# simdjson/simdjson-java

Hardware: AMD Instinct MI355X
Metric: GB/s JSON scanned (stage-1) (higher is better)
Workload: dtype u8; 1 GPU; twitter.json x6801 concatenated (north-star '4 GiB concatenated twitter.json'): stage-1 = UTF-8 validation + structural indexing + uint32 index compaction, one fused single-pass kernel; index count and status checked before and after the timed steps (the whole array against the oracle's closed form: --full); bytes_per_gpu=4294933515, structurals_per_gpu=375843663, tile_steps=auto, preheat_launches=40

## Files before the change

simdjson-java_amd/csrc/stage1.hip:

```cpp
#include <hip/hip_runtime.h>
#include <hip/hip_ext.h>
#include <stdint.h>

#include <type_traits>

#include "sj_block.h"
#include "sj_block32.h"
#include "sj_chain.h"
#include "stage1.h"

namespace sjmi {

__host__ __device__ constexpr uint32_t msad_const(int k, int base_weight_log2) {
    uint32_t r = 0;
    for (int i = 0; i < 4; ++i) {
        const int wgt = 1 << (base_weight_log2 + i);
        const int v = (1 << k) + wgt <= 255 ? (1 << k) + wgt : (1 << k) - wgt;
        r |= (uint32_t)v << (8 * i);
    }
    return r;
}

template <int K>
__device__ __forceinline__ sj_u64 plane_msad(const uint32_t w[16]) {
    constexpr uint32_t bit = 0x01010101u << K;
    constexpr uint32_t cA = msad_const(K, 0), cB = msad_const(K, 4);
    uint32_t half[2];
#pragma unroll
    for (int h = 0; h < 2; ++h) {
        uint32_t acc = 0;
#pragma unroll
        for (int j = 0; j < 4; ++j) {
            uint32_t v = __builtin_amdgcn_msad_u8(cA, w[8 * h + 2 * j] & bit, 0u);
            v = __builtin_amdgcn_msad_u8(cB, w[8 * h + 2 * j + 1] & bit, v);
            acc |= v << (8 * j);
        }
        half[h] = acc;
    }
    return (sj_u64)half[0] | ((sj_u64)half[1] << 32);
}

__device__ __forceinline__ void transpose_fast(const uint32_t w[16], sj_u64 p[8]) {
    p[0] = plane_msad<0>(w);
    p[1] = plane_msad<1>(w);
    p[2] = plane_msad<2>(w);
    p[3] = plane_msad<3>(w);
    p[4] = plane_msad<4>(w);
    p[5] = plane_msad<5>(w);
    p[6] = plane_msad<6>(w);
    p[7] = plane_msad<7>(w);
}

__global__ void k_transpose_selftest(const uint32_t* __restrict__ words, uint32_t nblocks, uint32_t* mismatches) {
    const uint32_t b = blockIdx.x * blockDim.x + threadIdx.x;
    if (b >= nblocks) return;
    uint32_t w[16];
#pragma unroll
    for (int i = 0; i < 16; ++i) w[i] = words[b * 16 + i];
    sj_u64 pf[8], pb[8], pr[8];
    transpose_fast(w, pf);
    sj_transpose_butterfly(w, pb);
    sj_transpose_ref(w, pr);
    uint32_t bad = 0;
#pragma unroll
    for (int k = 0; k < 8; ++k) bad += (pf[k] != pr[k]) + (pb[k] != pr[k]);
    if (bad) atomicAdd(mismatches, bad);
}

__device__ __forceinline__ uint32_t wave_sum(uint32_t v) {
#pragma unroll
    for (int d = 32; d >= 1; d >>= 1) v += __shfl_xor(v, d);
    return v;
}

__device__ __forceinline__ void publish_aggregate(sj_u64* tile_state, uint32_t tile, uint32_t T0, uint32_t T1,
                                                  uint32_t tpar, uint32_t errbits = 0) {
    granule_store(&tile_state[tile], CHAIN_AGG | ((sj_u64)errbits << 41) | ((sj_u64)tpar << 40) | ((sj_u64)T1 << 20) | (sj_u64)T0);
}
__device__ __forceinline__ void publish_prefix(sj_u64* tile_state, uint32_t tile, uint32_t par_after, sj_u64 cnt_after) {
    granule_store(&tile_state[tile], CHAIN_PFX | ((sj_u64)par_after << 40) | cnt_after);
}


template <int K>
__device__ __forceinline__ void tile_lookback(const sj_u64* tile_state, uint32_t tile, int lane, uint32_t* par_in,
                                              sj_u64* cnt_in, Stage1Result* res) {
    sj_u64 g0 = 0, g1 = 0;
    uint32_t gpar = 0;
    long long k = (long long)tile;
    uint32_t P = 0;
    sj_u64 C = 0;
    for (;;) {
        const long long hi = k - 1 - (long long)lane * K;
        sj_u64 v[K];
        int jp = K;
        int J = 64;
        for (uint32_t spins = 0;; ++spins) {
#pragma unroll
            for (int j = 0; j < K; ++j) v[j] = (hi - j >= 0) ? granule_load(&tile_state[hi - j]) : CHAIN_PFX;
            jp = K;
#pragma unroll
            for (int j = K - 1; j >= 0; --j)
                if ((v[j] >> 62) == 2) jp = j;
            bool ready = true;
#pragma unroll
            for (int j = 0; j < K; ++j)
                if (j < jp && v[j] == 0) ready = false;
            const sj_u64 pm = __ballot(jp < K);
            J = pm ? __builtin_ctzll(pm) : 64;
            const sj_u64 need = J >= 63 ? ~0ull : ((2ull << J) - 1ull);
            if ((__ballot(ready) & need) == need) break;
            if (spins > CHAIN_SPIN_LIMIT) {
                if (lane == 0)
                    __hip_atomic_fetch_or(&res->status, SJMI_ST_INTERNAL, __ATOMIC_RELAXED, __HIP_MEMORY_SCOPE_AGENT);
                break;
            }
            __builtin_amdgcn_s_sleep(1);
        }
        const int nin = lane < J ? K : (lane == J ? jp : 0);
        uint32_t c0 = 0, c1 = 0, lpar = 0;
        sj_u64 pfxv = 0;
#pragma unroll
        for (int j = K - 1; j >= 0; --j) {
            if (j == jp) pfxv = v[j];
            if (j < nin) {
                const uint32_t a0 = (uint32_t)v[j] & 0xFFFFFu, a1 = (uint32_t)(v[j] >> 20) & 0xFFFFFu;
                const uint32_t n0 = c0 + (lpar ? a1 : a0), n1 = c1 + (lpar ? a0 : a1);
                c0 = n0;
                c1 = n1;
                lpar ^= (uint32_t)(v[j] >> 40) & 1u;
            }
        }
        const sj_u64 pb = __ballot(lpar);
        const uint32_t q = (lane < 63) ? (uint32_t)__popcll(pb >> (lane + 1)) & 1u : 0u;
        const uint32_t w0 = wave_sum(q ? c1 : c0);
        const uint32_t w1 = wave_sum(q ? c0 : c1);
        const uint32_t wpar = (uint32_t)__popcll(pb) & 1u;
        if (J < 64) {
            const sj_u64 pv = __shfl(pfxv, J);
            P = (uint32_t)(pv >> 40) & 1u;
            C = pv & ((1ull << 40) - 1ull);
            C += P ? w1 : w0;
            P ^= wpar;
            C += P ? g1 : g0;
            P ^= gpar;
            break;
        }
        const sj_u64 n0 = (sj_u64)w0 + (wpar ? g1 : g0);
        const sj_u64 n1 = (sj_u64)w1 + (wpar ? g0 : g1);
        g0 = n0;
        g1 = n1;
        gpar ^= wpar;
        k -= 64 * K;
    }
    *par_in = P;
    *cnt_in = C;
}

__device__ __forceinline__ void single_doc_setup(const Stage1Single& ss, sj_u64 len, sj_u64 count, uint32_t status) {
    if (!ss.index_offsets) return;
    ss.doc_offsets[0] = 0;
    ss.doc_offsets[1] = len;
    ss.index_offsets[0] = 0;
    ss.index_offsets[1] = (status & (SJMI_ST_CAPACITY | SJMI_ST_INTERNAL)) ? 0ull : count;
    ss.doc_status[0] = status & 0xFFu;
    ss.doc_str_offsets[0] = 0;
    ss.doc_str_offsets[1] = 0;
    for (int i = 0; i < (int)(sizeof(WalkResult) / 4); ++i) ss.walk_result[i] = 0;
    for (int i = 0; i < 16; ++i) ss.slow_header[i] = 0;
}

constexpr int SCAN_K = 4;
struct Stage1Chain {
    static constexpr int K = SCAN_K;
    uint32_t* err;
    Stage1Result* res;
    uint32_t* out;
    sj_u64 out_cap;
    Stage1Result* result_out;
    const Stage1Single& ss;
    sj_u64 len;

    __device__ static void fold(const sj_u64 (&v)[K], uint32_t* c0, uint32_t* c1, uint32_t* par) {
        uint32_t a = 0, b = 0, lp = 0;
#pragma unroll
        for (int j = 0; j < K; ++j) {
            const uint32_t a0 = (uint32_t)v[j] & 0xFFFFFu, a1 = (uint32_t)(v[j] >> 20) & 0xFFFFFu;
            const uint32_t n0 = a + (lp ? a1 : a0), n1 = b + (lp ? a0 : a1);
            a = n0;
            b = n1;
            lp ^= (uint32_t)(v[j] >> 40) & 1u;
        }
        *c0 = a;
        *c1 = b;
        *par = lp;
    }
    __device__ static uint32_t errors(const sj_u64 (&v)[K], uint32_t q) {
        uint32_t e = 0;
#pragma unroll
        for (int j = 0; j < K; ++j) {
            if ((v[j] >> 41) & 1u) e |= SJMI_ST_UTF8;
            if ((v[j] >> 44) & 1u) e |= SJMI_ST_HALO;
            if ((v[j] >> (42 + q)) & 1u) e |= SJMI_ST_UNESCAPED;
            q ^= (uint32_t)(v[j] >> 40) & 1u;
        }
        return e;
    }
    __device__ void report(uint32_t e) const {
        if (__ballot(e != 0)) {
#pragma unroll
            for (int d = 32; d >= 1; d >>= 1) e |= __shfl_xor(e, d);
            if ((threadIdx.x & 63) == 0) __hip_atomic_fetch_or(err, e, __ATOMIC_RELAXED, __HIP_MEMORY_SCOPE_WORKGROUP);
        }
    }
    __device__ static void publish(const sj_u64 (&v)[K], sj_u64* pfx, sj_u64 first, uint32_t n, uint32_t q, sj_u64 run) {
#pragma unroll
        for (int j = 0; j < K; ++j) {
            run += q ? (uint32_t)(v[j] >> 20) & 0xFFFFFu : (uint32_t)v[j] & 0xFFFFFu;
            q ^= (uint32_t)(v[j] >> 40) & 1u;
            if (first + j < n) publish_prefix(pfx, (uint32_t)(first + j), q, run);
        }
    }

    struct Window {
        sj_u64 pb;
        uint32_t qrel;
        uint32_t mine0, mine1;
        uint32_t incl0, incl1;
        uint32_t tot0, tot1;
    };
    __device__ Window window(const sj_u64 (&v)[K], int lane) const {
        Window w;
        uint32_t c0, c1, lp;
        fold(v, &c0, &c1, &lp);
        w.pb = __ballot(lp);
        w.qrel = (uint32_t)__popcll(w.pb & ((1ull << lane) - 1ull)) & 1u;
        w.mine0 = w.qrel ? c1 : c0;
        w.mine1 = w.qrel ? c0 : c1;
        w.incl0 = wave_incl_add(w.mine0);
        w.incl1 = wave_incl_add(w.mine1);
        w.tot0 = (uint32_t)__builtin_amdgcn_readlane((int)w.incl0, 63);
        w.tot1 = (uint32_t)__builtin_amdgcn_readlane((int)w.incl1, 63);
        return w;
    }
    __device__ ChainState advance(ChainState in, const sj_u64 (&v)[K], const Window& w) const {
        report(errors(v, in.w ^ w.qrel));
        return {in.w ^ ((uint32_t)__popcll(w.pb) & 1u), in.c + (in.w ? w.tot1 : w.tot0)};
    }
    __device__ void publish_window(const sj_u64 (&v)[K], sj_u64* pfx, sj_u64 first, uint32_t n, ChainState in, const Window& w) const {
        publish(v, pfx, first, n, in.w ^ w.qrel, in.c + (in.w ? w.incl1 - w.mine1 : w.incl0 - w.mine0));
    }
    __device__ ChainState publish_ready(const sj_u64 (&v)[K], sj_u64* pfx, sj_u64 first, uint32_t n, int lane, bool act,
                                        ChainState s) const {
        uint32_t c0, c1, lp;
        fold(v, &c0, &c1, &lp);
        const sj_u64 pb = __ballot(act && lp);
        const uint32_t q = s.w ^ ((uint32_t)__popcll(pb & ((1ull << lane) - 1ull)) & 1u);
        const uint32_t mine = act ? (q ? c1 : c0) : 0u;
        const uint32_t incl = wave_incl_add(mine);
        if (act) publish(v, pfx, first, n, q, s.c + (incl - mine));
        report(act ? errors(v, q) : 0u);
        return {s.w ^ ((uint32_t)__popcll(pb) & 1u), s.c + (uint32_t)__builtin_amdgcn_readlane((int)incl, 63)};
    }
    __device__ void give_up() const {
        __hip_atomic_fetch_or(&res->status, SJMI_ST_INTERNAL, __ATOMIC_RELAXED, __HIP_MEMORY_SCOPE_AGENT);
        if (result_out) {
            result_out->count = 0;
            result_out->status = SJMI_ST_INTERNAL;
            result_out->reserved = 0;
            single_doc_setup(ss, len, 0, SJMI_ST_INTERNAL);
        }
    }
    __device__ void finish(ChainState s) const {
        res->count = s.c;
        uint32_t e = __hip_atomic_load(err, __ATOMIC_RELAXED, __HIP_MEMORY_SCOPE_WORKGROUP);
        if (s.w) e |= SJMI_ST_UNCLOSED;
        if (s.c < out_cap) out[s.c] = 0;
        else e |= SJMI_ST_CAPACITY;
        if (e) __hip_atomic_fetch_or(&res->status, e, __ATOMIC_RELAXED, __HIP_MEMORY_SCOPE_AGENT);
        if (result_out) {
            const uint32_t st_all = e | __hip_atomic_load(&res->status, __ATOMIC_RELAXED, __HIP_MEMORY_SCOPE_AGENT);
            result_out->count = s.c;
            result_out->status = st_all;
            result_out->reserved = 0;
            single_doc_setup(ss, len, s.c, st_all);
        }
    }
};


struct StepData {
    uint4 q0, q1, q2, q3;
    sj_u64 halo;
};

__device__ __forceinline__ void load_step(StepData& d, const uint8_t* __restrict__ buf, sj_u64 blk, sj_u64 nblocks, bool left_halo = false) {
    const sj_u64 b = blk < nblocks ? blk : nblocks - 1;
    const uint4* src = reinterpret_cast<const uint4*>(buf + b * 64);
    d.q0 = src[0];
    d.q1 = src[1];
    d.q2 = src[2];
    d.q3 = src[3];
    d.halo = *reinterpret_cast<const sj_u64*>(buf + ((b > 0 || left_halo) ? (long long)(b * 64) - 8 : 0ll));
}

constexpr uint32_t NO_TILE = 0xFFFFFFFFu;

__device__ __forceinline__ void zero_next_workspace(uint4* zero_ptr, uint32_t zero_chunks, uint32_t slot, uint32_t nslots,
                                                    int lane) {
    if (zero_ptr && nslots) {
        const uint32_t per = (zero_chunks + nslots - 1) / nslots;
        const uint32_t b = slot * per, e = b + per < zero_chunks ? b + per : zero_chunks;
        for (uint32_t i = b + (uint32_t)lane; i < e; i += 64) zero_ptr[i] = make_uint4(0, 0, 0, 0);
    }
}

constexpr uint32_t TICKET_CLASSES = 8;
constexpr int LB_K = 1;

#ifndef SJMI_S1_SORT_MIN
#define SJMI_S1_SORT_MIN 192
#endif
template <int S>
struct Parked {
    sj_u64 pot[S][64];
    sj_u64 m0[S][64];
    uint32_t meta[S][64];
};
template <int S, int LDSW>
union WaveShared {
    Parked<S> park;
    alignas(16) uint32_t stage[LDSW / 4];
    static_assert(sizeof(Parked<S>) <= LDSW, "LDS slice too small");
};

template <int S, int LDSW, bool SAFE, bool BATCH>
__device__ __forceinline__ void
stage1_body(const uint8_t* __restrict__ buf, sj_u64 len, uint32_t* __restrict__ out, sj_u64 out_cap,
            sj_u64* gstate, uint32_t* ticket, Stage1Result* res, uint32_t ngran, uint32_t dbg, uint4* zero_ptr,
            uint32_t zero_chunks, Stage1Result* result_out, sj_u64* __restrict__ blkpar, const uint32_t* __restrict__ skip,
            uint32_t* __restrict__ blkidx, uint16_t* __restrict__ blkw, uint4* zero2_ptr, uint32_t zero2_chunks, const Stage1Single& ss) {
    constexpr int E = S, CAP = LDSW / 4;
    if (skip && *skip) return;
    static_assert(S <= 4, "meta packs 14-bit offsets: at most 4 steps per granule");
    __shared__ WaveShared<S, LDSW> sh[4];
    __shared__ ChainHandoff hand;
    __shared__ uint32_t scan_err;
    const int lane = threadIdx.x & 63;
    const int wave = __builtin_amdgcn_readfirstlane(threadIdx.x >> 6);
    constexpr bool safe = SAFE;
    sj_u64* const agg = gstate;
    sj_u64* const pfx = gstate + ngran;
    const uint32_t my_cu = cu_id();
    uint32_t* const scanner_cu = reinterpret_cast<uint32_t*>(res) + WS_SCANNER_CU_WORD;
    if (!safe && blockIdx.x == 0) {
        if (threadIdx.x == 0) __hip_atomic_store(scanner_cu, my_cu, __ATOMIC_RELAXED, __HIP_MEMORY_SCOPE_AGENT);
        if ((dbg & DBG_FAKE_TIMEOUT) && threadIdx.x == 0)
            __hip_atomic_fetch_or(&res->status, SJMI_ST_INTERNAL, __ATOMIC_RELAXED, __HIP_MEMORY_SCOPE_AGENT);
        if (threadIdx.x == 0) {
            hand.seq = 0;
            hand.w = (dbg & FLAG_ENTRY_PARITY) ? 1u : 0u;
            hand.c = 0;
            scan_err = 0;
        }
        __syncthreads();
        if (!(dbg & DBG_NO_LOOKBACK)) {
            const Stage1Chain pol = {&scan_err, res, out, out_cap, result_out, ss, len};
            chain_scanner_wave(&hand, wave, lane, agg, pfx, ngran, pol);
        }
        return;
    }
    const uint32_t nworkers = (gridDim.x - (safe ? 0u : 1u)) * 4u;
    const uint32_t worker = (blockIdx.x - (safe ? 0u : 1u)) * 4u + (uint32_t)wave;
    WaveShared<S, LDSW>& ws = sh[wave];
    const uint32_t nblocks = (uint32_t)(len / 64) + ((dbg & FLAG_NO_TAIL) ? 0u : 1u);
    const uint32_t halo_blocks = dbg >> 16;
    const bool left_halo = halo_blocks != 0;
    const uint32_t entry_par = (dbg & FLAG_ENTRY_PARITY) ? 1u : 0u;
    const sj_u64 lt_mask = (1ull << lane) - 1ull;
    const uint32_t last = ngran - 1;

    const uint32_t NC = safe ? 1u : (nworkers < TICKET_CLASSES ? nworkers : TICKET_CLASSES);
    const uint32_t cls = worker % NC;
    uint32_t* const my_ticket = ticket + cls * 16u;
    uint32_t retire = 0;
    if (!safe && gridDim.x >= 64)
        retire = __hip_atomic_load(scanner_cu, __ATOMIC_RELAXED, __HIP_MEMORY_SCOPE_AGENT) ^ my_cu;
    else
        retire = 1;
    const bool first_by_ticket = safe || (dbg & FLAG_ALL_TICKETS) != 0;
    uint32_t cur;
    const uint32_t ticket_base = first_by_ticket ? 0u : (nworkers - cls + NC - 1u) / NC;
    if (first_by_ticket) cur = take_ticket(my_ticket) * NC + cls;
    else cur = worker;
    uint32_t prev = NO_TILE, prev_par = 0, prev_c0 = 0, prev_c1 = 0;
    uint32_t err = 0;
    StepData d;
    load_step(d, buf, cur * (64u * S) + (uint32_t)lane, nblocks, left_halo);

    for (;;) {
        const bool have = cur < ngran;
        uint32_t tk = 0;
        sj_u64 pfv = 0;
        sj_u64 pot[S], m[S];
        uint32_t meta[S];
        uint32_t wpar = 0, W0 = 0, WP = 0;
        auto request_ticket = [&] {
            if (lane == 0 && retire != 0) {
                uint32_t z = 0;
                asm volatile("" : "+v"(z));
                tk = __hip_atomic_fetch_add(my_ticket + z, 1u, __ATOMIC_RELAXED, __HIP_MEMORY_SCOPE_AGENT);
            }
        };
        auto request_prefix = [&] {
            uint32_t z = 0;
            asm volatile("" : "+v"(z));
            pfv = granule_load(&pfx[prev != NO_TILE && prev != 0 ? prev - 1 : 0u] + z);
        };
        auto next_granule = [&] {
            return retire != 0 ? ((uint32_t)__builtin_amdgcn_readfirstlane((int)tk) + ticket_base) * NC + cls : NO_TILE;
        };

        if (have) {
            __builtin_amdgcn_s_setprio(2);
            const uint32_t blk0 = cur * (64u * S);
            sj_u64 sm[S];
            uint32_t fl[S];
            uint32_t slow = 0;
            bool halo_short = false;
#pragma unroll
            for (int s = 0; s < S; ++s) {
                const uint32_t blk = blk0 + (uint32_t)s * 64u + (uint32_t)lane;
                const uint32_t w[16] = {d.q0.x, d.q0.y, d.q0.z, d.q0.w, d.q1.x, d.q1.y, d.q1.z, d.q1.w,
                                        d.q2.x, d.q2.y, d.q2.z, d.q2.w, d.q3.x, d.q3.y, d.q3.z, d.q3.w};
                const sj_u64 halo = d.halo;
                uint32_t plo[8], phi[8];
                sj_transpose32(w, plo, phi);
                asm volatile("" ::"v"(halo) : "memory");
                if (s + 1 < S) load_step(d, buf, blk0 + (uint32_t)(s + 1) * 64u + (uint32_t)lane, nblocks, left_halo);
                if (s == S - 1 && !safe) {
                    request_ticket();
                    request_prefix();
                }
                asm volatile("" ::: "memory");
                pot[s] = 0;
                sm[s] = 0;
                fl[s] = 0;
                bool unresolved = false;
                if (blk < nblocks) {
                    const bool has_halo = blk > 0 || left_halo;
                    uint32_t e_in = 0, p_in = 0;
                    if (has_halo) unresolved = !sj_carry_from_halo(halo, &e_in, &p_in);
                    if (blk0 + (uint32_t)s * 64u + 63u >= nblocks - 1u) {
                        const sj_u64 rem = len - (sj_u64)blk * 64;
                        sj_mask_tail32(plo, phi, rem < 64 ? (uint32_t)rem : 64u);
                    }
                    const uint32_t halo_hi = has_halo ? (uint32_t)(halo >> 32) & 0x80808080u : 0u;
                    const bool need_utf8 = __ballot((plo[7] | phi[7] | halo_hi) != 0) != 0;
                    SjUtf8Lazy uc = {0, 0};
                    if (need_utf8 && has_halo) uc = sj_utf8_carry_lazy(halo);
                    const SjBlockMasks32 bm = sj_block32(plo, phi, e_in, p_in, uc, need_utf8, BATCH, [](uint32_t x) { return __ballot(x != 0) != 0; });
                    pot[s] = ((sj_u64)bm.pot.hi << 32) | bm.pot.lo;
                    sm[s] = ((sj_u64)bm.sm0.hi << 32) | bm.sm0.lo;
                    fl[s] = bm.qpar | (min(bm.ue0, 1u) << 1) | (min(bm.ue1, 1u) << 2) | (min(bm.utf8, 1u) << 3);
                    if (BATCH) blkw[blk] = (uint16_t)bm.words;
                }
                slow |= unresolved ? (1u << s) : 0u;
            }
            if (__ballot(slow != 0)) {
                for (int s = 0; s < S; ++s) {
                    if (!((slow >> s) & 1u)) continue;
                    const sj_u64 blk = blk0 + (sj_u64)s * 64 + lane;
                    const sj_u64 start = blk * 64;
                    uint32_t w[16];
                    for (int i = 0; i < 16; ++i) w[i] = reinterpret_cast<const uint32_t*>(buf + start)[i];
                    const sj_u64 halo = *reinterpret_cast<const sj_u64*>(buf + start - 8);
                    uint32_t e_in = 0, p_in = 0;
                    sj_carry_slow(buf - (sj_u64)halo_blocks * 64, 0, start + (sj_u64)halo_blocks * 64, &e_in, &p_in);
                    if (left_halo && !(dbg & FLAG_HALO_FROM_START)) {
                        const uint8_t* hb = buf - (sj_u64)halo_blocks * 64;
                        const sj_u64 hs = start + (sj_u64)halo_blocks * 64;
                        if (sj_backslash_run_reaches(hb, 0, hb[hs - 1] == 0x22 ? hs - 1 : hs)) halo_short = true;
                    }
                    sj_u64 p[8];
                    sj_transpose_butterfly(w, p);
                    const sj_u64 rem = len - start;
                    sj_mask_tail(p, rem < 64 ? (uint32_t)rem : 64u);
                    const SjBlockMasks bm = sj_block(p, e_in, p_in, sj_utf8_carry(halo), true, nullptr, BATCH);
                    pot[s] = bm.pot;
                    sm[s] = bm.sm0;
                    fl[s] = bm.qpar | (bm.ue0 << 1) | (bm.ue1 << 2) | (bm.utf8 << 3);
                    if (BATCH && blk < nblocks) blkw[blk] = (uint16_t)bm.words;
                }
            }
            uint32_t gerr = 0;
#pragma unroll
            for (int s = 0; s < S; ++s) {
                const sj_u64 bal = __ballot(fl[s] & 1u);
                const uint32_t lp = ((uint32_t)__popcll(bal & lt_mask) & 1u) ^ wpar;
                wpar ^= (uint32_t)__popcll(bal) & 1u;
                m[s] = lp ? (pot[s] & sm[s]) : (pot[s] & ~sm[s]);
                const uint32_t c0 = (uint32_t)__popcll(m[s]), cp = (uint32_t)__popcll(pot[s]);
                const uint32_t packed = wave_incl_add(c0 | (cp << 16));
                const uint32_t tot = (uint32_t)__builtin_amdgcn_readlane((int)packed, 63);
                const uint32_t ex0 = W0 + (packed & 0xFFFFu) - c0;
                const uint32_t exp_ = WP + (packed >> 16) - cp;
                W0 += tot & 0xFFFFu;
                WP += tot >> 16;
                const uint32_t ue0 = (fl[s] >> 1) & 1u, ue1 = (fl[s] >> 2) & 1u;
                if (fl[s] & 8u) err |= SJMI_ST_UTF8;
                meta[s] = ex0 | (exp_ << 14) | ((lp ? ue1 : ue0) << 28) | ((lp ? ue0 : ue1) << 29) | (lp << 30);
                gerr |= ((fl[s] >> 3) & 1u) | ((meta[s] >> 27) & 6u);
            }
            uint32_t gbits = (__ballot(gerr & 1u) ? 1u : 0u) | (__ballot(gerr & 2u) ? 2u : 0u) | (__ballot(gerr & 4u) ? 4u : 0u);
            if (left_halo && __ballot(halo_short)) {
                gbits |= 8u;
                err |= SJMI_ST_HALO;
            }
            if (lane == 0 && !(dbg & DBG_NO_LOOKBACK)) {
                if (safe && cur == 0) publish_prefix(agg, 0, wpar ^ entry_par, (sj_u64)(entry_par ? WP - W0 : W0));
                else publish_aggregate(agg, cur, W0, WP - W0, wpar, gbits);
            }
            __builtin_amdgcn_s_setprio(0);
        }
        uint32_t nxt = NO_TILE;
        if (have) nxt = safe ? take_ticket(my_ticket) : next_granule();
        load_step(d, buf, nxt * (64u * S) + (uint32_t)lane, nblocks, left_halo);

        if (prev != NO_TILE) {
            uint32_t pe = entry_par;
            sj_u64 cnt_in = 0;
            if (dbg & DBG_NO_LOOKBACK) {
                cnt_in = (sj_u64)prev * 512ull * S;
            } else if (prev != 0) {
                if constexpr (safe) {
                    tile_lookback<LB_K>(agg, prev, lane, &pe, &cnt_in, res);
                } else {
                    sj_u64 pf = (sj_u64)(uint32_t)__builtin_amdgcn_readfirstlane((int)(uint32_t)pfv) |
                                ((sj_u64)(uint32_t)__builtin_amdgcn_readfirstlane((int)(uint32_t)(pfv >> 32)) << 32);
                    wait_prefix(&pfx[prev - 1], pf, [&] {
                        if (lane == 0) __hip_atomic_fetch_or(&res->status, SJMI_ST_INTERNAL, __ATOMIC_RELAXED, __HIP_MEMORY_SCOPE_AGENT);
                    });
                    pe = (uint32_t)(pf >> 40) & 1u;
                    cnt_in = pf & ((1ull << 40) - 1ull);
                }
            }
            const uint32_t WT_all = pe ? prev_c1 : prev_c0;
            if (safe && lane == 0 && !(dbg & DBG_NO_LOOKBACK)) {
                if (prev != 0) publish_prefix(agg, prev, pe ^ prev_par, cnt_in + WT_all);
                if (prev == last) {
                    const sj_u64 total = cnt_in + WT_all;
                    res->count = total;
                    uint32_t e = 0;
                    if (pe ^ prev_par) e |= SJMI_ST_UNCLOSED;
                    if (total < out_cap) out[total] = 0;
                    else e |= SJMI_ST_CAPACITY;
                    if (e) __hip_atomic_fetch_or(&res->status, e, __ATOMIC_RELAXED, __HIP_MEMORY_SCOPE_AGENT);
                }
            }
            const bool fits = cnt_in + WT_all < out_cap;
            if (!fits && WT_all) err |= SJMI_ST_CAPACITY;
            const sj_u64 pblk0 = (sj_u64)prev * (64 * S);
            uint32_t* stage = ws.stage;
#pragma unroll
            for (int g = 0; g < S / E; ++g) {
                sj_u64 mk[E];
                uint32_t pos[E];
                const uint32_t mb = ws.park.meta[g * E][0];
                const uint32_t gbase = pe ? ((mb >> 14) & 0x3FFFu) - (mb & 0x3FFFu) : (mb & 0x3FFFu);
                uint32_t gend = WT_all;
                if (g + 1 < S / E) {
                    const uint32_t me = ws.park.meta[(g + 1) * E][0];
                    gend = pe ? ((me >> 14) & 0x3FFFu) - (me & 0x3FFFu) : (me & 0x3FFFu);
                }
#pragma unroll
                for (int e = 0; e < E; ++e) {
                    const int s = g * E + e;
                    const sj_u64 pt = ws.park.pot[s][lane], mm = ws.park.m0[s][lane];
                    const uint32_t mt = ws.park.meta[s][lane];
                    mk[e] = pe ? (pt ^ mm) : mm;
                    const uint32_t o0 = mt & 0x3FFFu, op = (mt >> 14) & 0x3FFFu;
                    pos[e] = (pe ? op - o0 : o0) - gbase;
                    if (BATCH) blkidx[(pblk0 + (sj_u64)s * 64) + lane] = (uint32_t)(cnt_in + gbase) + pos[e];
                    if ((mt >> (28 + pe)) & 1u) err |= SJMI_ST_UNESCAPED;
                    if (blkpar) {
                        const sj_u64 pm = __ballot(((mt >> 30) ^ pe) & 1u);
                        if (lane == 0) blkpar[(sj_u64)prev * S + s] = pm;
                    }
                }
                wave_lds_fence();
                if (fits && !(dbg & DBG_NO_WRITE)) {
                    const uint32_t WT = gend - gbase;
                    uint32_t* dst0 = out + cnt_in + gbase;
                    auto flush_round = [&](uint32_t rbase, uint32_t rcount, uint32_t g0) {
                        const uint32_t span = g0 + rcount;
                        uint32_t* gbp = dst0 + rbase - g0;
                        for (uint32_t qi = lane; qi * 4 < span; qi += 64) {
                            const uint4 v = reinterpret_cast<const uint4*>(stage)[qi];
                            const uint32_t lo = qi * 4;
                            if (lo >= g0 && lo + 4 <= span) {
                                if constexpr (S == 4 && !BATCH) {
                                    typedef uint32_t u32x4_t __attribute__((ext_vector_type(4)));
                                    u32x4_t nv = {v.x, v.y, v.z, v.w};
                                    __builtin_nontemporal_store(nv, reinterpret_cast<u32x4_t*>(gbp) + qi);
                                } else {
                                    reinterpret_cast<uint4*>(gbp)[qi] = v;
                                }
                            } else {
                                if (lo + 0 >= g0 && lo + 0 < span) gbp[lo + 0] = v.x;
                                if (lo + 1 >= g0 && lo + 1 < span) gbp[lo + 1] = v.y;
                                if (lo + 2 >= g0 && lo + 2 < span) gbp[lo + 2] = v.z;
                                if (lo + 3 >= g0 && lo + 3 < span) gbp[lo + 3] = v.w;
                            }
                        }
                        wave_lds_fence();
                    };
                    auto fast_round = [&](uint32_t rbase, uint32_t rcount) {
                        const uint32_t g0 = (uint32_t)((cnt_in + gbase + rbase) & 3ull);
#pragma unroll
                        for (int e = 0; e < E; ++e) {
                            const uint32_t bstart = (uint32_t)((pblk0 + (sj_u64)(g * E + e) * 64 + lane) * 64);
                            uint32_t* q = stage + g0 + (pos[e] - rbase);
                            for (uint32_t lo = (uint32_t)mk[e]; lo; lo &= lo - 1) *q++ = bstart | (uint32_t)__builtin_ctz(lo);
                            for (uint32_t hi = (uint32_t)(mk[e] >> 32); hi; hi &= hi - 1)
                                *q++ = bstart | 32u | (uint32_t)__builtin_ctz(hi);
                        }
                        wave_lds_fence();
                        flush_round(rbase, rcount, g0);
                    };
                    auto sorted_round = [&](auto e0c, auto e1c, uint32_t rbase, uint32_t rcount) {
                        constexpr int E0 = decltype(e0c)::value, E1 = decltype(e1c)::value, NI = 2 * (E1 - E0);
                        static_assert(NI * 128 + 128 <= CAP, "the sort's tables overlay the staging slots");
                        const uint32_t g0 = (uint32_t)((cnt_in + gbase + rbase) & 3ull);
                        uint32_t* const hist = stage + NI * 128;
                        uint32_t* const bbase = hist + 64;
                        uint2* const items = reinterpret_cast<uint2*>(stage);
                        hist[lane] = 0u;
                        wave_lds_fence();
                        uint32_t hm[NI], cc[NI], rk[NI], inf[NI];
#pragma unroll
                        for (int e = E0; e < E1; ++e) {
                            const int i = 2 * (e - E0);
                            hm[i] = (uint32_t)mk[e];
                            hm[i + 1] = (uint32_t)(mk[e] >> 32);
                            cc[i] = (uint32_t)__popc(hm[i]);
                            cc[i + 1] = (uint32_t)__popc(hm[i + 1]);
                            const uint32_t p4 = (pos[e] - rbase + g0) * 4u;
                            const uint32_t ib = (uint32_t)(((g * E + e) * 64 + lane) * 64) << 16;
                            inf[i] = p4 | ib;
                            inf[i + 1] = (p4 + 4u * cc[i]) | (ib + (32u << 16));
                            rk[i] = atomicAdd(&hist[cc[i]], 1u);
                            rk[i + 1] = atomicAdd(&hist[cc[i + 1]], 1u);
                        }
                        wave_lds_fence();
                        const uint32_t hv = lane <= 32 ? hist[32 - lane] : 0u;
                        const uint32_t incl = wave_incl_add(hv);
                        if (lane <= 32) bbase[32 - lane] = incl - hv;
                        const uint32_t nz = (uint32_t)__builtin_amdgcn_readlane((int)incl, 31);
                        wave_lds_fence();
#pragma unroll
                        for (int i = 0; i < NI; ++i) items[bbase[cc[i]] + rk[i]] = make_uint2(hm[i], inf[i]);
                        wave_lds_fence();
                        const uint32_t trips = (nz + 63u) / 64u;
                        uint2 it[NI];
#pragma unroll
                        for (int r = 0; r < NI; ++r) it[r] = items[r * 64 + lane];
                        wave_lds_fence();
                        const uint32_t b32 = (uint32_t)(pblk0 * 64);
#pragma unroll
                        for (int r = 0; r < NI; ++r) {
                            if ((uint32_t)r >= trips) break;
                            uint32_t* q = reinterpret_cast<uint32_t*>(reinterpret_cast<char*>(stage) + (it[r].y & 0xFFFFu));
                            const uint32_t bv = b32 + (it[r].y >> 16);
                            uint32_t lo = it[r].x;
                            uint32_t* qh = q + __popc(lo) - 1;
                            while (lo) {
                                const uint32_t lz = (uint32_t)__builtin_clz(lo);
                                *q++ = bv | (uint32_t)__builtin_ctz(lo);
                                *qh-- = bv | (lz ^ 31u);
                                lo = lo & (lo - 1) & ~(0x80000000u >> lz);
                            }
                        }
                        wave_lds_fence();
                        flush_round(rbase, rcount, g0);
                    };
                    const uint32_t split = E >= 2 ? (uint32_t)__builtin_amdgcn_readfirstlane((int)pos[E / 2]) : 0u;
                    using std::integral_constant;
                    bool staged = false;
                    if (WT + 3 <= (uint32_t)CAP) {
                        if (WT > (uint32_t)(SJMI_S1_SORT_MIN * E)) sorted_round(integral_constant<int, 0>{}, integral_constant<int, E>{}, 0, WT);
                        else fast_round(0, WT);
                        staged = true;
                    }
                    if constexpr (E >= 2) {
                        if (!staged && split + 3 <= (uint32_t)CAP && WT - split + 3 <= (uint32_t)CAP) {
                            sorted_round(integral_constant<int, 0>{}, integral_constant<int, E / 2>{}, 0, split);
                            sorted_round(integral_constant<int, E / 2>{}, integral_constant<int, E>{}, split, WT - split);
                            staged = true;
                        }
                    }
                    if (!staged) {
                        for (uint32_t base = 0; base < WT; base += CAP) {
                            const uint32_t lim = base + CAP;
#pragma unroll
                            for (int e = 0; e < E; ++e) {
                                const uint32_t bstart = (uint32_t)((pblk0 + (sj_u64)(g * E + e) * 64 + lane) * 64);
                                uint32_t lo = (uint32_t)mk[e], hi = (uint32_t)(mk[e] >> 32);
                                uint32_t p2 = pos[e];
                                while (lo && p2 < lim) {
                                    stage[p2 - base] = bstart + (uint32_t)__builtin_ctz(lo);
                                    lo &= lo - 1;
                                    ++p2;
                                }
                                while (!lo && hi && p2 < lim) {
                                    stage[p2 - base] = bstart + 32u + (uint32_t)__builtin_ctz(hi);
                                    hi &= hi - 1;
                                    ++p2;
                                }
                                mk[e] = (sj_u64)lo | ((sj_u64)hi << 32);
                                pos[e] = p2;
                            }
                            wave_lds_fence();
                            const uint32_t nn = (WT - base) < (uint32_t)CAP ? (WT - base) : (uint32_t)CAP;
                            uint32_t* dst = dst0 + base;
                            for (uint32_t i = lane; i < nn; i += 64) dst[i] = stage[i];
                            wave_lds_fence();
                        }
                    }
                }
            }
        }
        if (!have) break;
        wave_lds_fence();
#pragma unroll
        for (int s = 0; s < S; ++s) {
            ws.park.pot[s][lane] = pot[s];
            ws.park.m0[s][lane] = m[s];
            ws.park.meta[s][lane] = meta[s];
        }
        wave_lds_fence();
        prev = cur;
        prev_par = wpar;
        prev_c0 = W0;
        prev_c1 = WP - W0;
        cur = nxt;
    }
#pragma unroll
    for (int dd = 32; dd >= 1; dd >>= 1) err |= __shfl_xor(err, dd);
    if (lane == 0 && err && !(dbg & DBG_NO_LOOKBACK))
        __hip_atomic_fetch_or(&res->status, err, __ATOMIC_RELAXED, __HIP_MEMORY_SCOPE_AGENT);
    zero_next_workspace(zero_ptr, zero_chunks, worker, nworkers, lane);
    zero_next_workspace(zero2_ptr, zero2_chunks, worker, nworkers, lane);
}

template <int S, int LDSW, bool SAFE, bool BATCH>
struct Stage1Kernel;
#ifndef SJMI_S1_PLAIN_WAVES
#define SJMI_S1_PLAIN_WAVES 4
#endif
template <int S, int LDSW, bool SAFE>
__global__ void __launch_bounds__(256)
#if SJMI_S1_PLAIN_WAVES
__attribute__((amdgpu_waves_per_eu(SJMI_S1_PLAIN_WAVES, SJMI_S1_PLAIN_WAVES)))
#endif
k_stage1(const uint8_t* __restrict__ buf, sj_u64 len, uint32_t* __restrict__ out, sj_u64 out_cap,
         sj_u64* gstate, uint32_t* ticket, Stage1Result* res, uint32_t ngran, uint32_t dbg, uint4* zero_ptr,
         uint32_t zero_chunks, Stage1Result* result_out, sj_u64* __restrict__ blkpar, const uint32_t* __restrict__ skip,
         uint32_t* __restrict__ blkidx, uint16_t* __restrict__ blkw, uint4* zero2_ptr, uint32_t zero2_chunks, Stage1Single ss) {
    stage1_body<S, LDSW, SAFE, false>(buf, len, out, out_cap, gstate, ticket, res, ngran, dbg, zero_ptr, zero_chunks, result_out, blkpar,
                                      skip, blkidx, blkw, zero2_ptr, zero2_chunks, ss);
}
#ifndef SJMI_S1_BATCH_WAVES
#define SJMI_S1_BATCH_WAVES 4
#endif
template <int S, int LDSW, bool SAFE>
__global__ void __launch_bounds__(256)
#if SJMI_S1_BATCH_WAVES
__attribute__((amdgpu_waves_per_eu(SJMI_S1_BATCH_WAVES, SJMI_S1_BATCH_WAVES)))
#endif
k_stage1_batch(const uint8_t* __restrict__ buf, sj_u64 len, uint32_t* __restrict__ out, sj_u64 out_cap,
               sj_u64* gstate, uint32_t* ticket, Stage1Result* res, uint32_t ngran, uint32_t dbg, uint4* zero_ptr,
               uint32_t zero_chunks, Stage1Result* result_out, sj_u64* __restrict__ blkpar, const uint32_t* __restrict__ skip,
               uint32_t* __restrict__ blkidx, uint16_t* __restrict__ blkw, uint4* zero2_ptr, uint32_t zero2_chunks, Stage1Single ss) {
    stage1_body<S, LDSW, SAFE, true>(buf, len, out, out_cap, gstate, ticket, res, ngran, dbg, zero_ptr, zero_chunks, result_out, blkpar,
                                     skip, blkidx, blkw, zero2_ptr, zero2_chunks, ss);
}
template <int S, int LDSW, bool SAFE>
struct Stage1Kernel<S, LDSW, SAFE, false> {
    static constexpr auto fn = k_stage1<S, LDSW, SAFE>;
};
template <int S, int LDSW, bool SAFE>
struct Stage1Kernel<S, LDSW, SAFE, true> {
    static constexpr auto fn = k_stage1_batch<S, LDSW, SAFE>;
};

static uint64_t granules_for(uint64_t len, int steps, bool no_tail = false) {
    const uint64_t nblocks = len / 64 + (no_tail ? 0 : 1);
    return (nblocks + 64ull * steps - 1) / (64ull * steps);
}

size_t stage1_workspace_bytes(uint64_t len, int steps) {
    return WS_TILE_STATE_OFFSET + 2 * (size_t)granules_for(len, steps) * sizeof(sj_u64);
}
Stage1Prefixes stage1_prefixes(const void* d_ws, uint64_t len, int steps) {
    Stage1Prefixes v;
    v.ngran = granules_for(len, steps);
    v.granule_bytes = (uint32_t)steps * 4096u;
    v.pfx = reinterpret_cast<const unsigned long long*>(static_cast<const uint8_t*>(d_ws) + WS_TILE_STATE_OFFSET) + v.ngran;
    return v;
}


int stage1_pick_steps(uint64_t len) {
    return len <= (4u << 20) ? 1 : (len <= (16u << 20) ? 2 : 4);
}

template <int S, int LDSW, bool SAFE, bool BATCH>
static hipError_t launch_mode(const uint8_t* d_buf, uint64_t len, uint32_t* d_out, uint64_t out_cap, sj_u64* gs,
                                 uint32_t* ticket, Stage1Result* res, uint64_t ngran, hipStream_t stream,
                                 hipEvent_t ev_start, hipEvent_t ev_stop, uint32_t dbg, const Stage1Extras& ex) {
    unsigned resident = 0;
    hipError_t e = resident_workgroups<Stage1Kernel<S, LDSW, SAFE, BATCH>::fn>(&resident);
    if (e != hipSuccess) return e;
    const uint64_t want = (ngran + 3) / 4 + (SAFE ? 0 : 1);
    if (dbg & DBG_SMALL_GRID) resident = SAFE ? 8 : 9;
    const dim3 grid((unsigned)(want < resident ? want : resident)), block(256);
    uint4* zp = static_cast<uint4*>(ex.zero_next);
    const uint32_t zc = (uint32_t)(ex.zero_bytes / 16);
    Stage1Result* ro = static_cast<Stage1Result*>(ex.result_out);
    sj_u64* bp = static_cast<sj_u64*>(ex.blkpar);
    uint32_t* bi = static_cast<uint32_t*>(ex.blkidx);
    uint16_t* bw = static_cast<uint16_t*>(ex.blkw);
    uint4* z2 = static_cast<uint4*>(ex.zero2);
    const uint32_t z2c = (uint32_t)(ex.zero2_bytes / 16);
    if (ev_start && ev_stop) {
        hipExtLaunchKernelGGL((Stage1Kernel<S, LDSW, SAFE, BATCH>::fn), grid, block, 0, stream, ev_start, ev_stop, 0, d_buf, (sj_u64)len,
                              d_out, (sj_u64)out_cap, gs, ticket, res, (uint32_t)ngran, dbg, zp, zc, ro, bp, ex.skip, bi, bw, z2, z2c, ex.single);
    } else {
        hipLaunchKernelGGL((Stage1Kernel<S, LDSW, SAFE, BATCH>::fn), grid, block, 0, stream, d_buf, (sj_u64)len, d_out, (sj_u64)out_cap,
                           gs, ticket, res, (uint32_t)ngran, dbg, zp, zc, ro, bp, ex.skip, bi, bw, z2, z2c, ex.single);
    }
    return hipGetLastError();
}

template <int S, int LDSW>
static hipError_t launch_variant(const uint8_t* d_buf, uint64_t len, uint32_t* d_out, uint64_t out_cap, sj_u64* gs,
                                 uint32_t* ticket, Stage1Result* res, uint64_t ngran, hipStream_t stream,
                                 hipEvent_t ev_start, hipEvent_t ev_stop, uint32_t dbg, const Stage1Extras& ex) {
    const bool batch = ex.blkidx && ex.blkw;
    if (dbg & FLAG_SAFE)
        return batch ? launch_mode<S, LDSW, true, true>(d_buf, len, d_out, out_cap, gs, ticket, res, ngran, stream, ev_start, ev_stop, dbg, ex)
                     : launch_mode<S, LDSW, true, false>(d_buf, len, d_out, out_cap, gs, ticket, res, ngran, stream, ev_start, ev_stop, dbg, ex);
    return batch ? launch_mode<S, LDSW, false, true>(d_buf, len, d_out, out_cap, gs, ticket, res, ngran, stream, ev_start, ev_stop, dbg, ex)
                 : launch_mode<S, LDSW, false, false>(d_buf, len, d_out, out_cap, gs, ticket, res, ngran, stream, ev_start, ev_stop, dbg, ex);
}

size_t stage1_block_entries(uint64_t len) { return (size_t)((len / 64 + 1 + 255) / 256 + 1) * 256; }

hipError_t stage1_launch(const uint8_t* d_buf, uint64_t len, uint32_t* d_out, uint64_t out_cap, void* d_ws,
                         int steps, hipStream_t stream, hipEvent_t ev_start, hipEvent_t ev_stop, uint32_t dbg, const Stage1Extras& ex) {
    const uint64_t ngran = granules_for(len, steps, (dbg & FLAG_NO_TAIL) != 0);
    if (ngran == 0) return hipErrorInvalidValue;
    const size_t ws_bytes = WS_TILE_STATE_OFFSET + 2 * (size_t)ngran * sizeof(sj_u64);
    hipError_t e = hipSuccess;
    if (!ex.workspace_is_zero && (e = hipMemsetAsync(d_ws, 0, ws_bytes, stream)) != hipSuccess) return e;
    uint8_t* ws = static_cast<uint8_t*>(d_ws);
    uint32_t* ticket = reinterpret_cast<uint32_t*>(ws + WS_TICKET_OFFSET);
    Stage1Result* res = reinterpret_cast<Stage1Result*>(ws + WS_RESULT_OFFSET);
    sj_u64* gs = reinterpret_cast<sj_u64*>(ws + WS_TILE_STATE_OFFSET);
    switch (steps) {
    case 1: e = launch_variant<1, 6144>(d_buf, len, d_out, out_cap, gs, ticket, res, ngran, stream, ev_start, ev_stop, dbg, ex); break;
    case 2: e = launch_variant<2, 9216>(d_buf, len, d_out, out_cap, gs, ticket, res, ngran, stream, ev_start, ev_stop, dbg, ex); break;
    case 4: e = launch_variant<4, 9216>(d_buf, len, d_out, out_cap, gs, ticket, res, ngran, stream, ev_start, ev_stop, dbg, ex); break;
    default: return hipErrorInvalidValue;
    }
    return e;
}

hipError_t transpose_selftest_launch(const uint32_t* d_words, uint32_t nblocks, uint32_t* d_mismatches,
                                     hipStream_t stream) {
    hipLaunchKernelGGL(k_transpose_selftest, dim3((nblocks + 255) / 256), dim3(256), 0, stream, d_words, nblocks,
                       d_mismatches);
    return hipGetLastError();
}

}
```

Baseline: 4126 GB/s.

## Defer last staged flush until after prefetched loads settle; batch blkpar stores

The final LDS-to-global flush of each granule's index writes is deferred until after the next step's input loads have been forced to complete, so the global loads and stores are ordered to overlap differently. The prefix readfirstlane is hoisted before the lookback. Per-block parity ballots are gathered into one lane per block and written by several lanes at once instead of serially from lane 0. This adds a static assert that there is one group per granule and keeps the staged data alive across the loop tail, which may raise register pressure.

```diff
diff --git a/simdjson-java_amd/csrc/stage1.hip b/simdjson-java_amd/csrc/stage1.hip
--- a/simdjson-java_amd/csrc/stage1.hip
+++ b/simdjson-java_amd/csrc/stage1.hip
@@ -397,6 +397,8 @@
     uint32_t err = 0;
     StepData d;
     load_step(d, buf, cur * (64u * S) + (uint32_t)lane, nblocks, left_halo);
+    auto settle_d = [&] { asm volatile("" ::"v"(d.q0.x), "v"(d.q1.x), "v"(d.q2.x), "v"(d.q3.x), "v"(d.halo) : "memory"); };
+    settle_d();
 
     for (;;) {
         const bool have = cur < ngran;
@@ -526,7 +528,41 @@
         uint32_t nxt = NO_TILE;
         if (have) nxt = safe ? take_ticket(my_ticket) : next_granule();
         load_step(d, buf, nxt * (64u * S) + (uint32_t)lane, nblocks, left_halo);
-
+        uint32_t pf_lo = 0, pf_hi = 0;
+        if constexpr (!safe) {
+            uint32_t vlo = (uint32_t)pfv, vhi = (uint32_t)(pfv >> 32);
+            asm volatile("" : "+v"(vlo), "+v"(vhi)::"memory");
+            pf_lo = (uint32_t)__builtin_amdgcn_readfirstlane((int)vlo);
+            pf_hi = (uint32_t)__builtin_amdgcn_readfirstlane((int)vhi);
+        }
+
+        static_assert(E == S, "one group per granule: the deferred round is the granule's last");
+        uint32_t* fl_gbp = nullptr;
+        uint32_t fl_span = 0, fl_g0 = 0;
+        auto flush_round = [&](uint32_t* gbp, uint32_t span, uint32_t g0) {
+            const uint32_t* stage = ws.stage;
+            uint32_t q0 = (uint32_t)lane;
+            asm volatile("" : "+v"(q0));
+            for (uint32_t qi = q0; qi * 4 < span; qi += 64) {
+                const uint4 v = reinterpret_cast<const uint4*>(stage)[qi];
+                const uint32_t lo = qi * 4;
+                if (lo >= g0 && lo + 4 <= span) {
+                    if constexpr (S == 4 && !BATCH) {
+                        typedef uint32_t u32x4_t __attribute__((ext_vector_type(4)));
+                        u32x4_t nv = {v.x, v.y, v.z, v.w};
+                        __builtin_nontemporal_store(nv, reinterpret_cast<u32x4_t*>(gbp) + qi);
+                    } else {
+                        reinterpret_cast<uint4*>(gbp)[qi] = v;
+                    }
+                } else {
+                    if (lo + 0 >= g0 && lo + 0 < span) gbp[lo + 0] = v.x;
+                    if (lo + 1 >= g0 && lo + 1 < span) gbp[lo + 1] = v.y;
+                    if (lo + 2 >= g0 && lo + 2 < span) gbp[lo + 2] = v.z;
+                    if (lo + 3 >= g0 && lo + 3 < span) gbp[lo + 3] = v.w;
+                }
+            }
+            wave_lds_fence();
+        };
         if (prev != NO_TILE) {
             uint32_t pe = entry_par;
             sj_u64 cnt_in = 0;
@@ -536,8 +572,7 @@
                 if constexpr (safe) {
                     tile_lookback<LB_K>(agg, prev, lane, &pe, &cnt_in, res);
                 } else {
-                    sj_u64 pf = (sj_u64)(uint32_t)__builtin_amdgcn_readfirstlane((int)(uint32_t)pfv) |
-                                ((sj_u64)(uint32_t)__builtin_amdgcn_readfirstlane((int)(uint32_t)(pfv >> 32)) << 32);
+                    sj_u64 pf = (sj_u64)pf_lo | ((sj_u64)pf_hi << 32);
                     wait_prefix(&pfx[prev - 1], pf, [&] {
                         if (lane == 0) __hip_atomic_fetch_or(&res->status, SJMI_ST_INTERNAL, __ATOMIC_RELAXED, __HIP_MEMORY_SCOPE_AGENT);
                     });
@@ -566,6 +601,7 @@
             for (int g = 0; g < S / E; ++g) {
                 sj_u64 mk[E];
                 uint32_t pos[E];
+                sj_u64 pmv = 0;
                 const uint32_t mb = ws.park.meta[g * E][0];
                 const uint32_t gbase = pe ? ((mb >> 14) & 0x3FFFu) - (mb & 0x3FFFu) : (mb & 0x3FFFu);
                 uint32_t gend = WT_all;
@@ -585,35 +621,23 @@
                     if ((mt >> (28 + pe)) & 1u) err |= SJMI_ST_UNESCAPED;
                     if (blkpar) {
                         const sj_u64 pm = __ballot(((mt >> 30) ^ pe) & 1u);
-                        if (lane == 0) blkpar[(sj_u64)prev * S + s] = pm;
+                        if (lane == s) pmv = pm;
                     }
                 }
+                if (blkpar && (uint32_t)(lane - g * E) < (uint32_t)E) blkpar[(sj_u64)prev * S + lane] = pmv;
                 wave_lds_fence();
                 if (fits && !(dbg & DBG_NO_WRITE)) {
                     const uint32_t WT = gend - gbase;
                     uint32_t* dst0 = out + cnt_in + gbase;
-                    auto flush_round = [&](uint32_t rbase, uint32_t rcount, uint32_t g0) {
-                        const uint32_t span = g0 + rcount;
+                    auto round_done = [&](uint32_t rbase, uint32_t rcount, uint32_t g0, bool last_round) {
                         uint32_t* gbp = dst0 + rbase - g0;
-                        for (uint32_t qi = lane; qi * 4 < span; qi += 64) {
-                            const uint4 v = reinterpret_cast<const uint4*>(stage)[qi];
-                            const uint32_t lo = qi * 4;
-                            if (lo >= g0 && lo + 4 <= span) {
-                                if constexpr (S == 4 && !BATCH) {
-                                    typedef uint32_t u32x4_t __attribute__((ext_vector_type(4)));
-                                    u32x4_t nv = {v.x, v.y, v.z, v.w};
-                                    __builtin_nontemporal_store(nv, reinterpret_cast<u32x4_t*>(gbp) + qi);
-                                } else {
-                                    reinterpret_cast<uint4*>(gbp)[qi] = v;
-                                }
-                            } else {
-                                if (lo + 0 >= g0 && lo + 0 < span) gbp[lo + 0] = v.x;
-                                if (lo + 1 >= g0 && lo + 1 < span) gbp[lo + 1] = v.y;
-                                if (lo + 2 >= g0 && lo + 2 < span) gbp[lo + 2] = v.z;
-                                if (lo + 3 >= g0 && lo + 3 < span) gbp[lo + 3] = v.w;
-                            }
+                        if (last_round) {
+                            fl_gbp = gbp;
+                            fl_span = g0 + rcount;
+                            fl_g0 = g0;
+                        } else {
+                            flush_round(gbp, g0 + rcount, g0);
                         }
-                        wave_lds_fence();
                     };
                     auto fast_round = [&](uint32_t rbase, uint32_t rcount) {
                         const uint32_t g0 = (uint32_t)((cnt_in + gbase + rbase) & 3ull);
@@ -626,9 +650,9 @@
                                 *q++ = bstart | 32u | (uint32_t)__builtin_ctz(hi);
                         }
                         wave_lds_fence();
-                        flush_round(rbase, rcount, g0);
+                        round_done(rbase, rcount, g0, true);
                     };
-                    auto sorted_round = [&](auto e0c, auto e1c, uint32_t rbase, uint32_t rcount) {
+                    auto sorted_round = [&](auto e0c, auto e1c, uint32_t rbase, uint32_t rcount, bool last_round) {
                         constexpr int E0 = decltype(e0c)::value, E1 = decltype(e1c)::value, NI = 2 * (E1 - E0);
                         static_assert(NI * 128 + 128 <= CAP, "the sort's tables overlay the staging slots");
                         const uint32_t g0 = (uint32_t)((cnt_in + gbase + rbase) & 3ull);
@@ -682,20 +706,20 @@
                             }
                         }
                         wave_lds_fence();
-                        flush_round(rbase, rcount, g0);
+                        round_done(rbase, rcount, g0, last_round);
                     };
                     const uint32_t split = E >= 2 ? (uint32_t)__builtin_amdgcn_readfirstlane((int)pos[E / 2]) : 0u;
                     using std::integral_constant;
                     bool staged = false;
                     if (WT + 3 <= (uint32_t)CAP) {
-                        if (WT > (uint32_t)(SJMI_S1_SORT_MIN * E)) sorted_round(integral_constant<int, 0>{}, integral_constant<int, E>{}, 0, WT);
+                        if (WT > (uint32_t)(SJMI_S1_SORT_MIN * E)) sorted_round(integral_constant<int, 0>{}, integral_constant<int, E>{}, 0, WT, true);
                         else fast_round(0, WT);
                         staged = true;
                     }
                     if constexpr (E >= 2) {
                         if (!staged && split + 3 <= (uint32_t)CAP && WT - split + 3 <= (uint32_t)CAP) {
-                            sorted_round(integral_constant<int, 0>{}, integral_constant<int, E / 2>{}, 0, split);
-                            sorted_round(integral_constant<int, E / 2>{}, integral_constant<int, E>{}, split, WT - split);
+                            sorted_round(integral_constant<int, 0>{}, integral_constant<int, E / 2>{}, 0, split, false);
+                            sorted_round(integral_constant<int, E / 2>{}, integral_constant<int, E>{}, split, WT - split, true);
                             staged = true;
                         }
                     }
@@ -730,6 +754,8 @@
                 }
             }
         }
+        settle_d();
+        if (fl_gbp) flush_round(fl_gbp, fl_span, fl_g0);
         if (!have) break;
         wave_lds_fence();
 #pragma unroll
```

Result: no change. 4141 GB/s, median of 6 (+0.4%).
